# annegnx/PnP-Flow

Measured on AMD Instinct MI355X. Metric: restored images/sec, higher is better.
Workload: dtype f32-equivalent (f16 hi+lo split operands, 3 x f16 MFMA per product, f32 accumulate); 1 GPU; CelebA-shaped 256x256 box-inpainting (half-size 40, sigma 0.05) pnp_flow B=32/GPU 100x5 (the configuration BASELINE.json's metric is quoted on; main.py:132-136 at 256^2); image=256x256x3, batch_per_gpu=32, global_batch=32, steps_pnp=100, num_samples=5, weights=synthetic seed 0 (no checkpoint offline), hipgraph=True, unet_batch=160, parallelism=dp1 (contiguous shards of the global batch, no data-path collective)

## Files before the change

### pnpflow_amd/csrc/conv_sp.hip

```cpp
#include <cstdlib>
#include "pp_common.h"

namespace pf {

constexpr int SP_PITCH = 20, SP_PW = 18;
constexpr int sp_rows(int MT) { return 8 * MT; }
constexpr int sp_npix(int MT) { return (sp_rows(MT) + 2) * SP_PW; }
constexpr int sp_patch(int MT) { return (sp_rows(MT) + 2) * SP_PITCH * 64; }
constexpr int sp_a9(int MT) { return (sp_npix(MT) * 4 + 255) / 256; }
constexpr int sp_tap(int NT, int TERMS = 3) { return (TERMS == 3 ? 2 : 1) * NT * 1024; }
constexpr int sp_x(int NT, int TERMS = 3) { return (5 * sp_tap(NT, TERMS) + 4095) / 4096 * 4096; }
constexpr int sp_y(int NT, int TERMS = 3) { return 4 * sp_tap(NT, TERMS); }
constexpr int SP_TAB = PP_MAXCH * 32;
constexpr int sp_lds(int MT, int NT, int TERMS = 3) { return sp_x(NT, TERMS) + sp_y(NT, TERMS) + 2 * sp_patch(MT) + SP_TAB; }
constexpr int sp_stage_n(int A9, int tap) {
    const int slot = tap < 4 ? tap : tap < 8 ? tap - 1 : 7;
    if (tap == 4 || tap == 8) return 0;
    return A9 / 7 + (slot < A9 % 7 ? 1 : 0);
}
constexpr int sp_stage_0(int A9, int tap) { int n = 0; for (int t = 0; t < tap; ++t) n += sp_stage_n(A9, t); return n; }

__device__ __forceinline__ void glds16_sp(unsigned voff, const char* sbase, unsigned lds_dst) {
    unsigned keep;
    asm volatile("s_mov_b32 %0, m0\n\ts_mov_b32 m0, %3\n\ts_nop 0\n\tglobal_load_lds_dwordx4 %1, %2\n\ts_mov_b32 m0, %0"
                 : "=&s"(keep) : "v"(voff), "s"(sbase), "s"(lds_dst) : "memory");
}

#ifdef PP_PROBE_BUILD
__device__ unsigned long long* g_sp_dbg = nullptr;
#define SP_STAMP(k) do { if (stamp_buf != nullptr && blockIdx.x == 0 && tid == 0 && stamp_n < 64) stamp_buf[stamp_n * 16 + (k)] = __builtin_readcyclecounter(); } while (0)
#else
#define SP_STAMP(k) do { } while (0)
#endif

template <int MT, int NT, bool RES, int TERMS = 3>
__global__ __launch_bounds__(256, 1) void conv_sp_kernel(const PPParams p) {
    constexpr int TH = sp_rows(MT), NPIX = sp_npix(MT), A9 = sp_a9(MT), PATCH = sp_patch(MT);
    constexpr int TAPB = sp_tap(NT, TERMS), XB = sp_x(NT, TERMS), COUT = 32 * NT, OB = COUT * 4;
    constexpr int NFRAG = (TERMS == 3 ? 2 : 1) * (MT + NT), NMMA = TERMS * MT * NT;
    static_assert(TERMS == 3 || TERMS == 1, "split terms");
    static_assert(sp_y(NT, TERMS) % 4096 == 0 && 9 * TAPB >= XB, "refill rounds of 4 KiB; slot X's over-fetch stays inside the chunk image");
    constexpr int REQ1 = sp_stage_0(A9, 4), REQ2 = A9 - REQ1 + 3;
    static_assert(sp_stage_0(A9, 9) == A9 && REQ1 + NT + 4 * MT * NT < 64, "staging distribution / vmcnt range");
    extern __shared__ __attribute__((aligned(16))) char smem[];
    const int tid = threadIdx.x;
    const int lane = tid & 63, wq = __builtin_amdgcn_readfirstlane(tid >> 6);
    const int l31 = lane & 31, hi = lane >> 5;
    constexpr unsigned PATCH0 = (unsigned)(XB + sp_y(NT, TERMS)), TAB = PATCH0 + 2u * (unsigned)PATCH;
    const pp_float_cptr scale_c = (pp_float_cptr)(uintptr_t)p.scale;
    const int nch = p.n9;

    const int qi = tid & 3, p0 = tid >> 2;
    unsigned pk[A9], ldsw[A9];
#pragma unroll
    for (int i = 0; i < A9; ++i) {
        const int pp = min(p0 + 64 * i, NPIX - 1);
        const int py = pp / SP_PW, px = pp - py * SP_PW;
        pk[i] = (unsigned)(py * p.W + px) | ((py == 0 ? 1u : 0u) << 20) | ((py == TH + 1 ? 1u : 0u) << 21) | ((px == 0 ? 1u : 0u) << 22) |
                ((px == SP_PW - 1 ? 1u : 0u) << 23);
        ldsw[i] = PATCH0 + (unsigned)((py * SP_PITCH + px) * 64) + (unsigned)((((qi >> 1) ^ ((px >> 2) & 3)) << 4) + (qi & 1) * 8);
    }
    const int pix_safe = p.W + 1;

    const int prow = l31 >> 4, pcol = l31 & 15;
    unsigned a_addr[3][2];
// ... 20 lines not shown
    const int rot = ntl > 0 ? (int)(((long)rg * p.rot) % ntl) : 0;
    auto tile_of = [&](int it) __attribute__((always_inline)) -> PPTile {
        const int idx = min(it, ntl - 1);
        const int wrapped = idx + rot >= ntl ? idx + rot - ntl : idx + rot;
        const int tl = t_begin + wrapped;
        PPTile r;
        const int tx = tl & ((1 << p.lx) - 1), ty = (tl >> p.lx) & ((1 << p.ly) - 1);
        r.b = tl >> (p.lx + p.ly); r.oy0 = ty * TH; r.ox0 = tx * 16;
        r.edge = (ty == 0 ? 1 : 0) | (ty == (1 << p.ly) - 1 ? 2 : 0) | (tx == 0 ? 4 : 0) | (tx == (1 << p.lx) - 1 ? 8 : 0);
        return r;
    };

    float4 ra[A9];
    unsigned zero_v;
    asm volatile("v_mov_b32 %0, 0" : "=v"(zero_v));
    struct Coef { float4 csc, csh; float ascale; unsigned inval; };
    Coef cf0, cf1;
    typedef const __attribute__((address_space(1))) char* gptr;
    struct Src { gptr base; unsigned cs4; };
    const unsigned q16 = (unsigned)qi * 16u;
    struct Desc { gptr base; const char* cb; unsigned cs4; int edge; unsigned sofs; };
    struct Ent { uint4 a, b; };
    auto fetch = [&](int c) __attribute__((always_inline)) -> Ent {
        Ent e;
        e.a = *reinterpret_cast<const uint4*>(smem + TAB + (unsigned)c * 32u); e.b = *reinterpret_cast<const uint4*>(smem + TAB + (unsigned)c * 32u + 16u);
        return e;
    };
    auto sptr = [&](unsigned lo, unsigned hi) __attribute__((always_inline)) -> gptr {
        return (gptr)(((unsigned long long)(unsigned)__builtin_amdgcn_readfirstlane((int)hi) << 32) | (unsigned)__builtin_amdgcn_readfirstlane((int)lo));
    };
    auto describe = [&](const PPTile& tl, const Ent& e) __attribute__((always_inline)) -> Desc {
        const int pix = (tl.b * p.H + tl.oy0) * p.W + tl.ox0 - p.W - 1;
        const int cstride = __builtin_amdgcn_readfirstlane((int)e.b.x), coff = __builtin_amdgcn_readfirstlane((int)e.b.y);
        const int gn_c0 = __builtin_amdgcn_readfirstlane((int)e.b.z), seg = __builtin_amdgcn_readfirstlane((int)e.b.w);
        Desc d;
        d.sofs = (unsigned)(8 * tl.b + seg) * 4u;
        d.edge = tl.edge;
        d.cb = reinterpret_cast<const char*>(p.coef + (tl.b * 2 * p.coef_stride + gn_c0));
        d.base = sptr(e.a.x, e.a.y) + (long)(pix * cstride + coff) * 4;
        d.cs4 = (unsigned)cstride * 4u;
        return d;
    };
    auto prep = [&](Coef& N, const Desc& d) __attribute__((always_inline)) -> Src {
        N.ascale = *reinterpret_cast<const float*>(reinterpret_cast<const char*>(p.scale) + d.sofs + zero_v);
        unsigned inval = 0;
#pragma unroll
        for (int i = 0; i < A9; ++i) inval |= (((pk[i] >> 20) & (unsigned)d.edge) != 0u ? 1u : 0u) << i;
        N.inval = inval;
        N.csc = *reinterpret_cast<const float4*>(d.cb + q16); N.csh = *reinterpret_cast<const float4*>(d.cb + (unsigned)(p.coef_stride * 4) + q16);
        Src r; r.base = d.base; r.cs4 = d.cs4;
        return r;
    };
    auto issue_one = [&](const Coef& N, const Src& sr, int i) __attribute__((always_inline)) {
        const unsigned px = ((N.inval >> i) & 1u) ? (unsigned)pix_safe : (pk[i] & 0xffffu);
        const pp_f4v t_ = *reinterpret_cast<const __attribute__((address_space(1))) pp_f4v*>(sr.base + (__umul24(px, sr.cs4) + q16));
        ra[i] = make_float4(t_.x, t_.y, t_.z, t_.w);
    };
    auto transform_one = [&](const Coef& S, int i, unsigned pofs) __attribute__((always_inline)) {
        float4 v = ra[i];
        v.x = silu_pp(v.x * S.csc.x + S.csh.x); v.y = silu_pp(v.y * S.csc.y + S.csh.y);
        v.z = silu_pp(v.z * S.csc.z + S.csh.z); v.w = silu_pp(v.w * S.csc.w + S.csh.w);
        const float f = ((S.inval >> i) & 1u) ? 0.0f : S.ascale;
        v.x *= f; v.y *= f; v.z *= f; v.w *= f;
        f16x4 h = {(_Float16)v.x, (_Float16)v.y, (_Float16)v.z, (_Float16)v.w};
        if constexpr (TERMS == 3) {
            f16x4 l = {(_Float16)(v.x - (float)h[0]), (_Float16)(v.y - (float)h[1]), (_Float16)(v.z - (float)h[2]), (_Float16)(v.w - (float)h[3])};
            const unsigned addr = ldsw[i] + pofs;
            *reinterpret_cast<f16x4*>(smem + addr) = h;
            *reinterpret_cast<f16x4*>(smem + (addr ^ 32u)) = l;
        } else {
            *reinterpret_cast<f16x4*>(smem + ldsw[i] + pofs) = h;
        }
    };

    f32x16 acc[MT][NT];
#pragma unroll
    for (int mt = 0; mt < MT; ++mt)
#pragma unroll
        for (int nt = 0; nt < NT; ++nt)
#pragma unroll
            for (int r = 0; r < 16; ++r) acc[mt][nt][r] = 0.f;
    float run1[4 * NT], run2[4 * NT];
#pragma unroll
    for (int j = 0; j < 4 * NT; ++j) { run1[j] = 0.f; run2[j] = 0.f; }
    int run_b = -1, run_n = 0;

    auto flush_stats = [&]() __attribute__((always_inline)) {
// ... 82 lines not shown
    auto load_tap = [&](int set, int tap, unsigned pofs) __attribute__((always_inline)) {
        const int ky = tap / 3, kx = tap % 3;
        const unsigned wb = (unsigned)(tap < 5 ? tap * TAPB : XB + (tap - 5) * TAPB) + b_lane;
        if constexpr (TERMS == 3) {
#pragma unroll
            for (int mt = 0; mt < MT; ++mt) fa[set][mt][1] = *reinterpret_cast<const f16x8*>(smem + a_addr[kx][1] + (unsigned)((mt * 2 + ky) * SP_PITCH * 64) + pofs);
        }
#pragma unroll
        for (int nt = 0; nt < NT; ++nt) fb[set][nt][0] = *reinterpret_cast<const f16x8*>(smem + wb + (unsigned)(nt * 1024));
#pragma unroll
        for (int mt = 0; mt < MT; ++mt) fa[set][mt][0] = *reinterpret_cast<const f16x8*>(smem + a_addr[kx][0] + (unsigned)((mt * 2 + ky) * SP_PITCH * 64) + pofs);
        if constexpr (TERMS == 3) {
#pragma unroll
            for (int nt = 0; nt < NT; ++nt) fb[set][nt][1] = *reinterpret_cast<const f16x8*>(smem + wb + (unsigned)(NT * 1024 + nt * 1024));
        }
    };
    auto load_frag = [&](int set, int tap, unsigned pofs, int idx) __attribute__((always_inline)) {
        const int ky = tap / 3, kx = tap % 3;
        const unsigned wb = (unsigned)(tap < 5 ? tap * TAPB : XB + (tap - 5) * TAPB) + b_lane;
        if constexpr (TERMS == 3) {
            if (idx < MT) fa[set][idx][1] = *reinterpret_cast<const f16x8*>(smem + a_addr[kx][1] + (unsigned)((idx * 2 + ky) * SP_PITCH * 64) + pofs);
            else if (idx < MT + NT) fb[set][idx - MT][0] = *reinterpret_cast<const f16x8*>(smem + wb + (unsigned)((idx - MT) * 1024));
            else if (idx < 2 * MT + NT) fa[set][idx - MT - NT][0] = *reinterpret_cast<const f16x8*>(smem + a_addr[kx][0] + (unsigned)(((idx - MT - NT) * 2 + ky) * SP_PITCH * 64) + pofs);
            else fb[set][idx - 2 * MT - NT][1] = *reinterpret_cast<const f16x8*>(smem + wb + (unsigned)(NT * 1024 + (idx - 2 * MT - NT) * 1024));
        } else {
            if (idx < NT) fb[set][idx][0] = *reinterpret_cast<const f16x8*>(smem + wb + (unsigned)(idx * 1024));
            else fa[set][idx - NT][0] = *reinterpret_cast<const f16x8*>(smem + a_addr[kx][0] + (unsigned)(((idx - NT) * 2 + ky) * SP_PITCH * 64) + pofs);
        }
    };
    auto mma_group = [&](int set, int g) __attribute__((always_inline)) {
// ... 45 lines not shown
                acc[mt][nt] = __builtin_amdgcn_mfma_f32_32x32x16_f16(fa[set][mt][term == 0 ? 1 : 0], fb[set][nt][term == 1 ? 1 : 0], acc[mt][nt], 0, 0, 0);
                __builtin_amdgcn_sched_barrier(0);
                const int j = g * NT + nt;
                if (j < nrounds) {
                    if ((j & 3) == 0) asm volatile("s_mov_b32 m0, %0\n\ts_nop 0" :: "s"(dst0 + (unsigned)(j * 1024)) : "memory");
                    if ((j & 3) == 0) asm volatile("global_load_lds_dwordx4 %0, %1" :: "v"(b_lane), "s"(sb + j * 1024) : "memory");
                    if ((j & 3) == 1) asm volatile("global_load_lds_dwordx4 %0, %1 offset:1024" :: "v"(b_lane), "s"(sb + (j - 1) * 1024) : "memory");
                    if ((j & 3) == 2) asm volatile("global_load_lds_dwordx4 %0, %1 offset:2048" :: "v"(b_lane), "s"(sb + (j - 2) * 1024) : "memory");
                    if ((j & 3) == 3) asm volatile("global_load_lds_dwordx4 %0, %1 offset:3072" :: "v"(b_lane), "s"(sb + (j - 3) * 1024) : "memory");
                }
                if (j < NFRAG) load_frag(nset, ntap, npofs, j);
                __builtin_amdgcn_sched_barrier(0);
            }
        }
        asm volatile("s_mov_b32 m0, %0" :: "s"(keep));
    };

    int stamp_n = 0; (void)stamp_n;
#ifdef PP_PROBE_BUILD
    unsigned long long* const stamp_buf = g_sp_dbg;
#endif
    gptr wimg_next = (gptr)(uintptr_t)p.ch[1].wimg;
    Desc dn;
    Src sr;
    auto chunk = [&](int it, int c, auto SI_, bool last_chunk) __attribute__((always_inline)) {
        constexpr int SI = decltype(SI_)::value;
        constexpr unsigned PCUR = SI ? PATCH : 0, PNXT = SI ? 0 : PATCH;
        Coef& C = SI == 0 ? cf1 : cf0;
        Coef& N = SI == 0 ? cf0 : cf1;
        const gptr wnext = wimg_next;
// ... 15 lines not shown
        else asm volatile("s_waitcnt vmcnt(%0) lgkmcnt(0)" :: "n"(REQ1) : "memory");
#pragma unroll
        for (int i = REQ1; i < A9; ++i) asm volatile("" :: "v"(ra[i].x));
        SP_STAMP(13);
        __builtin_amdgcn_s_barrier();
        __builtin_amdgcn_sched_barrier(0);
        SP_STAMP(5);
        mma_tap_refill((4 + SI) & 1, wnext, 0, XB / 4096, (5 + SI) & 1, 5, PCUR);
        SP_STAMP(6);
#pragma unroll
        for (int tap = 5; tap < 8; ++tap) {
            __builtin_amdgcn_sched_barrier(0);
            int q = c + 3, wrap = 0;
            if (q >= nch) { q -= nch; wrap = 1; }
            if (q >= nch) { q -= nch; wrap = 2; }
            const int c2 = c + 2 >= nch ? c + 2 - nch : c + 2;
            Ent eq, e2;
            if (tap == 6) { eq = fetch(q); e2 = fetch(c2); }
            load_tap((tap + 1 + SI) & 1, tap + 1, PCUR);
#pragma unroll
            for (int i = sp_stage_0(A9, tap); i < sp_stage_0(A9, tap) + sp_stage_n(A9, tap); ++i) { transform_one(C, i, PNXT); issue_one(N, sr, i); }
            if (tap == 6) {
                dn = describe(tile_of(it + wrap), eq);
                wimg_next = sptr(e2.a.z, e2.a.w);
            }
            if (tap == 7) sr = prep(C, dn);
            mma_tap((tap + SI) & 1);
            tap_pattern();
            __builtin_amdgcn_sched_barrier(0);
            SP_STAMP(2 + tap);
        }
        __builtin_amdgcn_sched_barrier(0);
        asm volatile("s_waitcnt vmcnt(%0) lgkmcnt(0)" :: "n"(REQ2) : "memory");
#pragma unroll
        for (int i = 0; i < REQ1; ++i) asm volatile("" :: "v"(ra[i].x));
        SP_STAMP(14);
        __builtin_amdgcn_s_barrier();
        __builtin_amdgcn_sched_barrier(0);
        SP_STAMP(10);
        mma_tap_refill((8 + SI) & 1, wnext, 5, 4 * TAPB / 4096, (9 + SI) & 1, 0, PNXT);
        SP_STAMP(11);
        SP_STAMP(12);
        ++stamp_n;
    };

    if (ntl <= 0) return;
    for (int c = 0; c < nch; ++c) {
        if (tid == 0) {
            const unsigned long long sp_ = (unsigned long long)(uintptr_t)p.ch[c].src, wp_ = (unsigned long long)(uintptr_t)p.ch[c].wimg;
            *reinterpret_cast<uint4*>(smem + TAB + (unsigned)c * 32u) = make_uint4((unsigned)sp_, (unsigned)(sp_ >> 32), (unsigned)wp_, (unsigned)(wp_ >> 32));
            *reinterpret_cast<uint4*>(smem + TAB + (unsigned)c * 32u + 16u) = make_uint4((unsigned)p.ch[c].cstride, (unsigned)p.ch[c].coff, (unsigned)p.ch[c].gn_c0, (unsigned)p.ch[c].seg);
        }
    }
    __syncthreads();
    {
        const Src s0 = prep(cf0, describe(tile_of(0), fetch(0)));
#pragma unroll
        for (int i = 0; i < A9; ++i) issue_one(cf0, s0, i);
        {
            const char* w0 = reinterpret_cast<const char*>(p.ch[0].wimg);
#pragma unroll
            for (int j = 0; j < (TERMS == 3 ? 9 * TAPB : XB) / 4096; ++j) glds16_sp(dma_lane, w0 + j * 4096, (unsigned)(j * 4096) + (unsigned)(wq * 1024));
            if constexpr (TERMS != 3) {
#pragma unroll
                for (int j = 0; j < 4 * TAPB / 4096; ++j) glds16_sp(dma_lane, w0 + 5 * TAPB + j * 4096, (unsigned)(XB + j * 4096) + (unsigned)(wq * 1024));
            }
        }
#pragma unroll
        for (int i = 0; i < A9; ++i) transform_one(cf0, i, 0);
        const Src s1 = prep(cf1, describe(tile_of(0), fetch(1)));
#pragma unroll
        for (int i = 0; i < A9; ++i) issue_one(cf1, s1, i);
        sr = prep(cf0, describe(tile_of(2 >= nch ? 1 : 0), fetch(2 >= nch ? 2 - nch : 2)));
        asm volatile("s_waitcnt vmcnt(0) lgkmcnt(0)" ::: "memory");
        __builtin_amdgcn_s_barrier();
        __builtin_amdgcn_sched_barrier(0);
        load_tap(0, 0, 0);
    }
    const int seg_lo[4] = {0, seg_c1 > 0 ? seg_c1 : nch, seg_c2 > 0 ? seg_c2 : nch, nch};
#pragma unroll 1
    for (int it = 0; it < ntl; ++it) {
        tile_inputs(tile_of(it));
#pragma unroll 1
        for (int sg = 0; sg < 3; ++sg) {
            const int lo = seg_lo[sg], hi = seg_lo[sg + 1];
            if (lo >= hi) continue;
            if (sg > 0) {
                const PPTile tl = tile_of(it);
                const float ratio = scale_c[8 * tl.b + seg_id[sg]] * scale_c[8 * tl.b + 4 + seg_id[sg - 1]];
                if (ratio != 1.0f) {
#pragma unroll
                    for (int mt = 0; mt < MT; ++mt)
#pragma unroll
                        for (int nt = 0; nt < NT; ++nt)
#pragma unroll
                            for (int r = 0; r < 16; ++r) acc[mt][nt][r] *= ratio;
                }
// ... 4 lines not shown
                chunk(it, c + 1, ic<1>{}, false);
            }
        }
        epilogue(tile_of(it));
    }
    flush_stats();
    asm volatile("s_waitcnt vmcnt(0)" ::: "memory");
}


static int ilog2_exact_sp(int v) { int l = 0; while ((1 << l) < v) ++l; return (1 << l) == v ? l : -1; }

bool conv_sp_supported(const ConvParams& p, int stride, int up, int terms) {
    static const int mode = getenv("PNPFLOW_HIP_SP") ? atoi(getenv("PNPFLOW_HIP_SP")) : 1;
    if (mode == 0 || (terms != 3 && !(terms == 1 && mode != 3)) || stride != 1 || up != 0 || p.gnb_x != nullptr) return false;
    if (p.Cout != 128 && !(p.Cout == 64 && mode == 1)) return false;
    if (p.out_cstride != p.Cout || (p.residual != nullptr && p.res_cstride != p.Cout)) return false;
    if (p.addvec == nullptr) return false;
    const int TH = p.Cout == 128 ? sp_rows(2) : sp_rows(4);
    if (p.H % TH || p.W % 16 || p.Hs != p.H || p.Ws != p.W) return false;
    if ((TH + 1) * p.W + SP_PW - 1 > 65535) return false;
    if (ilog2_exact_sp(p.H / TH) < 0 || ilog2_exact_sp(p.W / 16) < 0) return false;
    const int grid = persistent_grid();
    if (grid < 8 || (long)p.B * (p.H / TH) * (p.W / 16) < 4L * grid) return false;
    int nch = 0;
    for (int i = 0; i < p.nseg; ++i) {
        const ConvSeg& s = p.seg[i];
        if ((double)p.B * p.H * p.W * s.cstride >= 2147483648.0) return false;
        if (s.w_mode != 0 || s.w16 == nullptr || s.C % 32 || s.taps != 9 || s.xform != 2) return false;
        nch += s.C / 16;
    }
    if (nch < 2 || nch > PP_MAXCH || (nch & 1)) return false;
    return p.gn_C > 0 && p.coef != nullptr && p.scale != nullptr;
}

template <int MT, int NT, int TERMS>
static hipError_t launch_sp_t(const PPParams& p0, hipStream_t s) {
    static unsigned long long attr_set[2] = {0ull, 0ull};
    const bool res = p0.residual != nullptr;
    const void* kern = res ? reinterpret_cast<const void*>(conv_sp_kernel<MT, NT, true, TERMS>) : reinterpret_cast<const void*>(conv_sp_kernel<MT, NT, false, TERMS>);
    { hipError_t e = set_max_dynamic_lds_once(kern, attr_set[res ? 1 : 0], 160 * 1024); if (e != hipSuccess) return e; }
    const int grid = persistent_grid();
    if (grid <= 0) return hipErrorInvalidConfiguration;
    PPParams p = p0;
    p.lx = ilog2_exact_sp(p.W / 16); p.ly = ilog2_exact_sp(p.H / sp_rows(MT));
    p.rot = 5;
    if (res) hipLaunchKernelGGL((conv_sp_kernel<MT, NT, true, TERMS>), dim3(grid), dim3(256), sp_lds(MT, NT, TERMS), s, p);
    else hipLaunchKernelGGL((conv_sp_kernel<MT, NT, false, TERMS>), dim3(grid), dim3(256), sp_lds(MT, NT, TERMS), s, p);
    return hipGetLastError();
}

hipError_t launch_conv_sp(const PPParams& p0, hipStream_t s, int terms) {
    if (p0.n9 < 2 || (p0.n9 & 1) || p0.n1 != 0 || (terms != 3 && terms != 1)) return hipErrorInvalidValue;
    if (p0.cout == 128) return terms == 3 ? launch_sp_t<2, 4, 3>(p0, s) : launch_sp_t<2, 4, 1>(p0, s);
    if (p0.cout == 64) return terms == 3 ? launch_sp_t<4, 2, 3>(p0, s) : launch_sp_t<4, 2, 1>(p0, s);
    return hipErrorInvalidValue;
}

}
```

### pnpflow_amd/csrc/engine.hip

```cpp
#include <algorithm>
#include <cmath>
#include <cstdio>
#include <cstring>
#include <cstdlib>
#include <functional>
#include <map>
#include <memory>
#include <string>
#include <vector>

#include "../../include/pnpflow_hip.h"
#include "pf_common.h"
#include "weight_pack.h"

using namespace pf;

namespace {

struct HostTensor { std::vector<int64_t> shape; std::vector<float> data; bool loaded = false; };

struct ResDesc {
    std::string prefix;
    int cin0 = 0, cin1 = 0;
    int cout = 0;
// ... 408 lines not shown
    if (!sp && !(p.Cout == 32 && conv_pp_supported(p, stride, up, terms))) return 0;
    q = PPParams{};
    q.cout = p.Cout;
    const int kc = sp ? 16 : 32;
    int n = 0;
    for (int i = 0; i < p.nseg; ++i) {
        const ConvSeg& sg = p.seg[i];
        auto it = e->w16_src.find(sg.w16);
        if (it == e->w16_src.end()) return 0;
        for (int cc = 0; cc < sg.C / kc; ++cc) {
            PPChunk& k = q.ch[n++];
            k.src = sg.src; k.cstride = sg.cstride; k.coff = sg.coff + cc * kc; k.xform = sg.xform;
            k.gn_c0 = sg.gn_off + cc * kc; k.seg = i;
            const std::string& wn = it->second.name; const int lo = it->second.lo + cc * kc;
            const wpack::Oihw w = oihw(e, wn);
            if (w.O != p.Cout || (sp && w.kk != 9)) return 0;
            k.wimg = !sp ? weight_image(e, wn + "#pp" + std::to_string(lo), [&] { return wpack::chunk_pp(w, lo); })
                         : weight_image(e, wn + (terms == 1 ? "#sph" : "#sp") + std::to_string(p.Cout) + "_" + std::to_string(lo), [&] { return wpack::chunk_sp(w, lo, p.Cout / 32, terms); });
            if (!k.wimg) return 0;
            (sg.taps == 9 ? q.n9 : q.n1) += 1;
        }
    }
    q.B = p.B; q.H = p.H; q.W = p.W;
    q.out = p.out; q.addvec = p.addvec; q.addvec_bs = p.addvec_bs; q.residual = p.residual; q.res_scale = p.res_scale;
    q.stats_out = p.stats_out; q.out_scale = p.out_scale; q.coef = p.coef; q.coef_stride = p.coef_stride; q.scale = p.scale;
    return sp ? 2 : 1;
}

static void push_conv(Builder& bd, const ConvParams& p0, int stride = 1, int up = 0) {
    ConvParams p = with_coef(bd, p0, bd.plan->ops);
    Op op{}; op.kind = OP_CONV; op.terms = conv_terms(bd.e);
    op.use_pp = attach_pp(bd, p, stride, up, op.ppp);
// ... 1435 lines not shown

int pf_engine_profile_read(pf_engine* e, int64_t* launches, double* ms_conv_gemm, double* flops_conv_gemm) {
    if (!e) return PF_ERR_INVALID;
    HIPCHK(e, hipDeviceSynchronize());
    FILE* dump = getenv("PNPFLOW_HIP_PROFILE_CSV") ? fopen(getenv("PNPFLOW_HIP_PROFILE_CSV"), "w") : nullptr;
    if (dump) fprintf(dump, "idx,H,W,Cout,K,nseg,taps0,stride,up,gflop,us,tflops,dma,alg_mb\n");
    for (size_t i = 0; i < e->ev_used; ++i) {
        float ms = 0.f;
        if (hipEventElapsedTime(&ms, e->ev_pool[i].first, e->ev_pool[i].second) == hipSuccess) { e->prof_ms += ms; e->prof_launches += 1; }
        if (dump && i < e->ev_ops.size() && e->ev_ops[i]) {
            const Op& op = *e->ev_ops[i]; size_t K = 0;
            for (int j = 0; j < op.cp.nseg; ++j) K += (size_t)op.cp.seg[j].taps * op.cp.seg[j].C;
            double bytes = (double)op.cp.B * op.cp.H * op.cp.W * op.cp.Cout * 4.0 * (op.cp.residual ? 2.0 : 1.0);
            for (int j = 0; j < op.cp.nseg; ++j) bytes += (double)op.cp.B * op.cp.Hs * op.cp.Ws * op.cp.seg[j].C * 4.0;
            fprintf(dump, "%zu,%d,%d,%d,%zu,%d,%d,%d,%d,%.4f,%.2f,%.2f,%d,%.3f", i, op.cp.H, op.cp.W, op.cp.Cout, K, op.cp.nseg, op.cp.seg[0].taps,
                    op.stride, op.up, op.flops / 1e9, ms * 1e3, op.flops / (ms * 1e-3) / 1e12, op.use_pp == 2 ? 5 : op.use_pp ? 2 : op.dma, bytes / 1e6);
            fprintf(dump, "\n");
        }
    }
    if (dump) fclose(dump);
    e->ev_used = 0;
    if (launches) *launches = e->prof_launches;
    if (ms_conv_gemm) *ms_conv_gemm = e->prof_ms;
    if (flops_conv_gemm) *flops_conv_gemm = e->prof_flops;
    return PF_OK;
}

}

#include "engine_dflow.inc"
```

### pnpflow_amd/csrc/pf_common.h

```cpp
#pragma once
#include <hip/hip_runtime.h>
#include <stdint.h>
#include <atomic>

namespace pf {

inline hipError_t set_max_dynamic_lds_once(const void* kernel, unsigned long long& done, int bytes = 160 * 1024) {
    int dev = 0;
    hipError_t e = hipGetDevice(&dev);
    if (e != hipSuccess) return e;
    if (dev >= 0 && dev < 64 && ((done >> dev) & 1ull)) return hipSuccess;
    e = hipFuncSetAttribute(kernel, hipFuncAttributeMaxDynamicSharedMemorySize, bytes);
    if (e == hipSuccess && dev >= 0 && dev < 64) done |= 1ull << dev;
    return e;
}

inline int device_cu_count() {
    static std::atomic<int> cache[64] = {};
    int dev = 0;
    if (hipGetDevice(&dev) != hipSuccess) return 0;
    if (dev >= 0 && dev < 64) { const int c = cache[dev].load(std::memory_order_relaxed); if (c > 0) return c; }
    int v = 0;
    if (hipDeviceGetAttribute(&v, hipDeviceAttributeMultiprocessorCount, dev) != hipSuccess || v < 0) v = 0;
    if (dev >= 0 && dev < 64) cache[dev].store(v, std::memory_order_relaxed);
// ... 109 lines not shown
hipError_t launch_gn_coef(const GnCoefParams& p, int B, hipStream_t s);

struct PrepParams {
    const float* src[3]; void* dst[3];
    int C[3], cstride[3], coff[3], xform[3], gn_off[3];
    int nseg, B, Hs, Ws, terms;
    const float* coef; int coef_stride;
    const float* scale;
};
hipError_t launch_prep_split(const PrepParams& p, hipStream_t s);
bool conv_dma_supported(const ConvParams& p, int stride, int up, int terms);
bool conv_dma_phase_shape_ok(const ConvParams& p, int terms);
hipError_t launch_conv_dma(const ConvParams& p, int up, hipStream_t s, int terms);
size_t conv_dma_a16_bytes(int B, int C, int Hs, int Ws, int terms);

constexpr int PP_MAXCH = 24;
struct PPChunk {
    const float* src;
    const void* wimg;
    int cstride, coff;
    int xform;
    int gn_c0;
    int seg;
    int pad_;
};
struct PPParams {
    PPChunk ch[PP_MAXCH];
    int n9, n1;
    int cout;
    int B, H, W, lx, ly;
    int rot;
// ... 102 lines not shown
```

### pnpflow_amd/csrc/weight_pack.h

```cpp
#pragma once
#include <cstddef>
#include <vector>

namespace wpack {

using half_t = _Float16;
constexpr int KC = 16;

struct Oihw {
    const float* w; int O, I, kk;
    float operator()(int o, int i, int tap) const { return w[((size_t)o * I + i) * kk + tap]; }
};

struct Split { half_t hi, lo; half_t part(int p) const { return p ? lo : hi; } };
inline Split split16(float w) { w *= 256.0f; const half_t hi = (half_t)w; return {hi, (half_t)(w - (float)hi)}; }

inline int col_channel(int n) { return 4 * (n & 7) + (n >> 3); }

inline std::vector<float> frag32(const Oihw& w, int lo, int hi) {
    const int C = hi - lo, nchunk = (C + KC - 1) / KC;
    std::vector<float> img((size_t)nchunk * w.kk * w.O * KC, 0.f);
    for (int c = 0; c < C; ++c)
        for (int tap = 0; tap < w.kk; ++tap)
            for (int n = 0; n < w.O; ++n)
// ... 27 lines not shown
}

inline std::vector<half_t> chunk_sp(const Oihw& w, int lo, int NT, int terms) {
    const int P = terms == 1 ? 1 : 2;
    std::vector<half_t> img((size_t)w.kk * P * NT * 512, (half_t)0.f);
    size_t at = 0;
    for (int tap = 0; tap < w.kk; ++tap)
        for (int part = 0; part < P; ++part)
            for (int nt = 0; nt < NT; ++nt)
                for (int kh = 0; kh < 2; ++kh)
                    for (int n = 0; n < 32; ++n)
                        for (int i = 0; i < 8; ++i) img[at++] = split16(w(32 * nt + col_channel(n), lo + 8 * kh + i, tap)).part(part);
    return img;
}

inline std::vector<half_t> edge_frag(const Oihw& w, bool begin) {
    const int cimg = begin ? w.I : w.O;
    std::vector<half_t> img((size_t)2 * 2 * 64 * 8, (half_t)0.f);
    for (int ks = 0; ks < 2; ++ks) for (int hh = 0; hh < 2; ++hh) for (int n = 0; n < 32; ++n) for (int j = 0; j < 8; ++j) {
        const int k = begin ? 16 * ks + 8 * hh + j : n;
        if (k >= 9 * cimg) continue;
        const Split s = begin ? split16(w(n, k / 9, k % 9)) : split16(w(n % cimg, 16 * hh + 8 * ks + j, n / cimg));
        for (int part = 0; part < 2; ++part) img[((((size_t)ks * 2 + part) * 2 + hh) * 32 + n) * 8 + j] = s.part(part);
    }
    return img;
}

inline std::vector<float> adjoint(const Oihw& w, int lo, int hi) {
    const int C = hi - lo;
    std::vector<float> t((size_t)C * w.O * w.kk);
// ... 21 lines not shown
```

Baseline: 3.300 images/s.

## Fuse 1x1 shortcut conv into the streaming 3x3 conv kernel

Adds a shortcut-carrying variant of the persistent 3x3 conv kernel. It appends the 1x1 shortcut segment's raw-input chunks after the 3x3 chunks, which extends the ResNet block fusion so the shortcut conv no longer needs a separate pass or launch. The 1x1 weights stream through an LDS ring. Raw inputs skip the GN/SiLU transform through a per-chunk flag, and the accumulator is rescaled between segments. Small global-to-LDS touch loads are issued during the 3x3 taps, apparently to prefetch shortcut inputs into cache. This adds LDS use, kernel complexity and a rescaling step that can affect precision.

Measured after the change: 3.307 images/s (median of 6 runs). About the same (+0.2%).

```diff
diff --git a/pnpflow_amd/csrc/conv_sp.hip b/pnpflow_amd/csrc/conv_sp.hip
--- a/pnpflow_amd/csrc/conv_sp.hip
+++ b/pnpflow_amd/csrc/conv_sp.hip
@@ -13,6 +13,12 @@
 constexpr int sp_y(int NT, int TERMS = 3) { return 4 * sp_tap(NT, TERMS); }
 constexpr int SP_TAB = PP_MAXCH * 32;
 constexpr int sp_lds(int MT, int NT, int TERMS = 3) { return sp_x(NT, TERMS) + sp_y(NT, TERMS) + 2 * sp_patch(MT) + SP_TAB; }
+constexpr int SP_RING = 4, SP_TOUCH = 1024;
+constexpr int sp_lds_sc(int MT, int NT) { return sp_lds(MT, NT, 3) + SP_RING * sp_tap(NT, 3) + SP_TOUCH; }
+#ifndef SP_TOUCH_PAIRS_N
+#define SP_TOUCH_PAIRS_N 2
+#endif
+constexpr int SP_TOUCH_PAIRS = SP_TOUCH_PAIRS_N;
 constexpr int sp_stage_n(int A9, int tap) {
     const int slot = tap < 4 ? tap : tap < 8 ? tap - 1 : 7;
     if (tap == 4 || tap == 8) return 0;
@@ -25,30 +31,40 @@
     asm volatile("s_mov_b32 %0, m0\n\ts_mov_b32 m0, %3\n\ts_nop 0\n\tglobal_load_lds_dwordx4 %1, %2\n\ts_mov_b32 m0, %0"
                  : "=&s"(keep) : "v"(voff), "s"(sbase), "s"(lds_dst) : "memory");
 }
+__device__ __forceinline__ void glds4_sp(unsigned voff, const __attribute__((address_space(1))) char* sbase, unsigned lds_dst) {
+    unsigned keep;
+    asm volatile("s_mov_b32 %0, m0\n\ts_mov_b32 m0, %3\n\ts_nop 0\n\tglobal_load_lds_dword %1, %2\n\ts_mov_b32 m0, %0"
+                 : "=&s"(keep) : "v"(voff), "s"(sbase), "s"(lds_dst) : "memory");
+}
 
 #ifdef PP_PROBE_BUILD
 __device__ unsigned long long* g_sp_dbg = nullptr;
+__device__ int g_sp_touch_off = 0;
 #define SP_STAMP(k) do { if (stamp_buf != nullptr && blockIdx.x == 0 && tid == 0 && stamp_n < 64) stamp_buf[stamp_n * 16 + (k)] = __builtin_readcyclecounter(); } while (0)
 #else
 #define SP_STAMP(k) do { } while (0)
 #endif
 
-template <int MT, int NT, bool RES, int TERMS = 3>
+template <int MT, int NT, bool RES, int TERMS = 3, bool SC = false>
 __global__ __launch_bounds__(256, 1) void conv_sp_kernel(const PPParams p) {
+    static_assert(!SC || (TERMS == 3 && !RES), "the shortcut-carrying form: default precision, no identity residual");
     constexpr int TH = sp_rows(MT), NPIX = sp_npix(MT), A9 = sp_a9(MT), PATCH = sp_patch(MT);
     constexpr int TAPB = sp_tap(NT, TERMS), XB = sp_x(NT, TERMS), COUT = 32 * NT, OB = COUT * 4;
     constexpr int NFRAG = (TERMS == 3 ? 2 : 1) * (MT + NT), NMMA = TERMS * MT * NT;
     static_assert(TERMS == 3 || TERMS == 1, "split terms");
     static_assert(sp_y(NT, TERMS) % 4096 == 0 && 9 * TAPB >= XB, "refill rounds of 4 KiB; slot X's over-fetch stays inside the chunk image");
-    constexpr int REQ1 = sp_stage_0(A9, 4), REQ2 = A9 - REQ1 + 3;
+    constexpr int NTOUCH = SC ? SP_TOUCH_PAIRS * (TH * 16 / 256) : 0;
+    constexpr int REQ1 = sp_stage_0(A9, 4), REQ2 = A9 - REQ1 + 3 + NTOUCH;
     static_assert(sp_stage_0(A9, 9) == A9 && REQ1 + NT + 4 * MT * NT < 64, "staging distribution / vmcnt range");
     extern __shared__ __attribute__((aligned(16))) char smem[];
     const int tid = threadIdx.x;
     const int lane = tid & 63, wq = __builtin_amdgcn_readfirstlane(tid >> 6);
     const int l31 = lane & 31, hi = lane >> 5;
     constexpr unsigned PATCH0 = (unsigned)(XB + sp_y(NT, TERMS)), TAB = PATCH0 + 2u * (unsigned)PATCH;
+    constexpr unsigned W1 = TAB + (unsigned)SP_TAB, TOUCH = W1 + (unsigned)(SP_RING * TAPB);
     const pp_float_cptr scale_c = (pp_float_cptr)(uintptr_t)p.scale;
-    const int nch = p.n9;
+    const int n9 = p.n9;
+    const int nch = SC ? p.n9 + p.n1 : p.n9;
 
     const int qi = tid & 3, p0 = tid >> 2;
     unsigned pk[A9], ldsw[A9];
@@ -99,12 +115,12 @@
     float4 ra[A9];
     unsigned zero_v;
     asm volatile("v_mov_b32 %0, 0" : "=v"(zero_v));
-    struct Coef { float4 csc, csh; float ascale; unsigned inval; };
+    struct Coef { float4 csc, csh; float ascale; unsigned inval; float lk; };
     Coef cf0, cf1;
     typedef const __attribute__((address_space(1))) char* gptr;
     struct Src { gptr base; unsigned cs4; };
     const unsigned q16 = (unsigned)qi * 16u;
-    struct Desc { gptr base; const char* cb; unsigned cs4; int edge; unsigned sofs; };
+    struct Desc { gptr base; const char* cb; unsigned cs4; int edge; unsigned sofs; int raw; };
     struct Ent { uint4 a, b; };
     auto fetch = [&](int c) __attribute__((always_inline)) -> Ent {
         Ent e;
@@ -117,8 +133,10 @@
     auto describe = [&](const PPTile& tl, const Ent& e) __attribute__((always_inline)) -> Desc {
         const int pix = (tl.b * p.H + tl.oy0) * p.W + tl.ox0 - p.W - 1;
         const int cstride = __builtin_amdgcn_readfirstlane((int)e.b.x), coff = __builtin_amdgcn_readfirstlane((int)e.b.y);
-        const int gn_c0 = __builtin_amdgcn_readfirstlane((int)e.b.z), seg = __builtin_amdgcn_readfirstlane((int)e.b.w);
+        const int gn_c0 = __builtin_amdgcn_readfirstlane((int)e.b.z), segw = __builtin_amdgcn_readfirstlane((int)e.b.w);
+        const int seg = SC ? (segw & 0xff) : segw;
         Desc d;
+        d.raw = SC ? (segw >> 8) & 1 : 0;
         d.sofs = (unsigned)(8 * tl.b + seg) * 4u;
         d.edge = tl.edge;
         d.cb = reinterpret_cast<const char*>(p.coef + (tl.b * 2 * p.coef_stride + gn_c0));
@@ -126,13 +144,20 @@
         d.cs4 = (unsigned)cstride * 4u;
         return d;
     };
-    auto prep = [&](Coef& N, const Desc& d) __attribute__((always_inline)) -> Src {
+    auto prep = [&](Coef& N, const Desc& d, auto SEL_) __attribute__((always_inline)) -> Src {
         N.ascale = *reinterpret_cast<const float*>(reinterpret_cast<const char*>(p.scale) + d.sofs + zero_v);
         unsigned inval = 0;
 #pragma unroll
         for (int i = 0; i < A9; ++i) inval |= (((pk[i] >> 20) & (unsigned)d.edge) != 0u ? 1u : 0u) << i;
         N.inval = inval;
         N.csc = *reinterpret_cast<const float4*>(d.cb + q16); N.csh = *reinterpret_cast<const float4*>(d.cb + (unsigned)(p.coef_stride * 4) + q16);
+        if constexpr (SC && decltype(SEL_)::value == 0) N.lk = 0.0f;
+        if constexpr (SC && decltype(SEL_)::value != 0) {
+            const bool rw = d.raw != 0;
+            N.csc.x = rw ? 1.0f : N.csc.x; N.csc.y = rw ? 1.0f : N.csc.y; N.csc.z = rw ? 1.0f : N.csc.z; N.csc.w = rw ? 1.0f : N.csc.w;
+            N.csh.x = rw ? 0.0f : N.csh.x; N.csh.y = rw ? 0.0f : N.csh.y; N.csh.z = rw ? 0.0f : N.csh.z; N.csh.w = rw ? 0.0f : N.csh.w;
+            N.lk = rw ? -__builtin_inff() : 0.0f;
+        }
         Src r; r.base = d.base; r.cs4 = d.cs4;
         return r;
     };
@@ -143,8 +168,14 @@
     };
     auto transform_one = [&](const Coef& S, int i, unsigned pofs) __attribute__((always_inline)) {
         float4 v = ra[i];
-        v.x = silu_pp(v.x * S.csc.x + S.csh.x); v.y = silu_pp(v.y * S.csc.y + S.csh.y);
-        v.z = silu_pp(v.z * S.csc.z + S.csh.z); v.w = silu_pp(v.w * S.csc.w + S.csh.w);
+        if constexpr (SC) {
+            auto silu_lk = [&](float u) __attribute__((always_inline)) -> float { return u * __builtin_amdgcn_rcpf(1.0f + __builtin_amdgcn_exp2f(__builtin_fmaf(u, -1.44269504088896340736f, S.lk))); };
+            v.x = silu_lk(v.x * S.csc.x + S.csh.x); v.y = silu_lk(v.y * S.csc.y + S.csh.y);
+            v.z = silu_lk(v.z * S.csc.z + S.csh.z); v.w = silu_lk(v.w * S.csc.w + S.csh.w);
+        } else {
+            v.x = silu_pp(v.x * S.csc.x + S.csh.x); v.y = silu_pp(v.y * S.csc.y + S.csh.y);
+            v.z = silu_pp(v.z * S.csc.z + S.csh.z); v.w = silu_pp(v.w * S.csc.w + S.csh.w);
+        }
         const float f = ((S.inval >> i) & 1u) ? 0.0f : S.ascale;
         v.x *= f; v.y *= f; v.z *= f; v.w *= f;
         f16x4 h = {(_Float16)v.x, (_Float16)v.y, (_Float16)v.z, (_Float16)v.w};
@@ -156,6 +187,17 @@
         } else {
             *reinterpret_cast<f16x4*>(smem + ldsw[i] + pofs) = h;
         }
+    };
+
+    auto transform_raw = [&](const Coef& S, int i, unsigned pofs) __attribute__((always_inline)) {
+        float4 v = ra[i];
+        const float f = ((S.inval >> i) & 1u) ? 0.0f : S.ascale;
+        v.x *= f; v.y *= f; v.z *= f; v.w *= f;
+        f16x4 h = {(_Float16)v.x, (_Float16)v.y, (_Float16)v.z, (_Float16)v.w};
+        f16x4 l = {(_Float16)(v.x - (float)h[0]), (_Float16)(v.y - (float)h[1]), (_Float16)(v.z - (float)h[2]), (_Float16)(v.w - (float)h[3])};
+        const unsigned addr = ldsw[i] + pofs;
+        *reinterpret_cast<f16x4*>(smem + addr) = h;
+        *reinterpret_cast<f16x4*>(smem + (addr ^ 32u)) = l;
     };
 
     f32x16 acc[MT][NT];
@@ -268,6 +310,17 @@
 #pragma unroll
             for (int nt = 0; nt < NT; ++nt) fb[set][nt][1] = *reinterpret_cast<const f16x8*>(smem + wb + (unsigned)(NT * 1024 + nt * 1024));
         }
+    };
+    auto load_tap1 = [&](int set, unsigned wslot, unsigned pofs) __attribute__((always_inline)) {
+        const unsigned wb = wslot + b_lane;
+#pragma unroll
+        for (int mt = 0; mt < MT; ++mt) fa[set][mt][1] = *reinterpret_cast<const f16x8*>(smem + a_addr[1][1] + (unsigned)((mt * 2 + 1) * SP_PITCH * 64) + pofs);
+#pragma unroll
+        for (int nt = 0; nt < NT; ++nt) fb[set][nt][0] = *reinterpret_cast<const f16x8*>(smem + wb + (unsigned)(nt * 1024));
+#pragma unroll
+        for (int mt = 0; mt < MT; ++mt) fa[set][mt][0] = *reinterpret_cast<const f16x8*>(smem + a_addr[1][0] + (unsigned)((mt * 2 + 1) * SP_PITCH * 64) + pofs);
+#pragma unroll
+        for (int nt = 0; nt < NT; ++nt) fb[set][nt][1] = *reinterpret_cast<const f16x8*>(smem + wb + (unsigned)(NT * 1024 + nt * 1024));
     };
     auto load_frag = [&](int set, int tap, unsigned pofs, int idx) __attribute__((always_inline)) {
         const int ky = tap / 3, kx = tap % 3;
@@ -343,6 +396,26 @@
             }
         }
         asm volatile("s_mov_b32 m0, %0" :: "s"(keep));
+    };
+
+    auto touch = [&](int it, int c) __attribute__((always_inline)) {
+        const PPTile tl = tile_of(it);
+        const int pix = (tl.b * p.H + tl.oy0) * p.W + tl.ox0;
+        const int last = (p.n1 >> 1) - 1;
+#pragma unroll
+        for (int k = 0; k < SP_TOUCH_PAIRS; ++k) {
+            const Ent e = fetch(n9 + 2 * min(1 + SP_TOUCH_PAIRS * c + k, last));
+            const int cstride = __builtin_amdgcn_readfirstlane((int)e.b.x), coff = __builtin_amdgcn_readfirstlane((int)e.b.y);
+            const gptr base = sptr(e.a.x, e.a.y) + (long)(pix * cstride + coff) * 4;
+#pragma unroll
+            for (int i = 0; i < TH * 16 / 256; ++i) {
+                unsigned voff = __umul24((unsigned)(((tid >> 4) + 16 * i) * p.W + (tid & 15)), (unsigned)cstride * 4u);
+#ifdef PP_PROBE_BUILD
+                if (g_sp_touch_off) voff = 0u;
+#endif
+                glds4_sp(voff, base, TOUCH + (unsigned)(wq * 256));
+            }
+        }
     };
 
     int stamp_n = 0; (void)stamp_n;
@@ -388,9 +461,10 @@
             int q = c + 3, wrap = 0;
             if (q >= nch) { q -= nch; wrap = 1; }
             if (q >= nch) { q -= nch; wrap = 2; }
-            const int c2 = c + 2 >= nch ? c + 2 - nch : c + 2;
+            const int c2 = c + 2 >= n9 ? c + 2 - n9 : c + 2;
             Ent eq, e2;
             if (tap == 6) { eq = fetch(q); e2 = fetch(c2); }
+            if constexpr (SC) { if (tap == 5) touch(it, c); }
             load_tap((tap + 1 + SI) & 1, tap + 1, PCUR);
 #pragma unroll
             for (int i = sp_stage_0(A9, tap); i < sp_stage_0(A9, tap) + sp_stage_n(A9, tap); ++i) { transform_one(C, i, PNXT); issue_one(N, sr, i); }
@@ -398,7 +472,7 @@
                 dn = describe(tile_of(it + wrap), eq);
                 wimg_next = sptr(e2.a.z, e2.a.w);
             }
-            if (tap == 7) sr = prep(C, dn);
+            if (tap == 7) sr = prep(C, dn, ic<1>{});
             mma_tap((tap + SI) & 1);
             tap_pattern();
             __builtin_amdgcn_sched_barrier(0);
@@ -418,17 +492,68 @@
         ++stamp_n;
     };
 
+    int ring_n = 0;
+    auto chunk1 = [&](int it, int g, auto SI_) __attribute__((always_inline)) {
+        constexpr int SI = decltype(SI_)::value;
+        constexpr unsigned PNXT = SI ? 0 : PATCH;
+        constexpr int NREG = 3 * MT * NT / 2;
+        Coef& C = SI == 0 ? cf1 : cf0;
+        Coef& N = SI == 0 ? cf0 : cf1;
+        static_assert(!SC || A9 + 2 <= NREG, "one float4 of the next chunk is staged per two MFMAs of the tap");
+        const bool next_raw = g + 1 < nch;
+        int q = g + 3, wrap = 0;
+        if (q >= nch) { q -= nch; wrap = 1; }
+        if (q >= nch) { q -= nch; wrap = 2; }
+        int jn = g - n9 + SP_RING;
+        if (jn >= p.n1) jn -= p.n1;
+        if (jn >= p.n1) jn -= p.n1;
+        Ent eq, ew;
+        SP_STAMP(0);
+#pragma unroll
+        for (int gi = 0; gi < NREG; ++gi) {
+            __builtin_amdgcn_sched_barrier(0);
+            if (gi == 0) { eq = fetch(q); ew = fetch(n9 + jn); }
+#pragma unroll
+            for (int k = 2 * gi; k < 2 * gi + 2; ++k) {
+                const int grp = k / NT, nt = k % NT, term = grp / MT, mt = grp % MT;
+                acc[mt][nt] = __builtin_amdgcn_mfma_f32_32x32x16_f16(fa[SI][mt][term == 0 ? 1 : 0], fb[SI][nt][term == 1 ? 1 : 0], acc[mt][nt], 0, 0, 0);
+            }
+            if (gi < A9) {
+                if (next_raw) transform_raw(C, gi, PNXT); else transform_one(C, gi, PNXT);
+                issue_one(N, sr, gi);
+            }
+            if (gi == A9) dn = describe(tile_of(it + wrap), eq);
+            if (gi == A9 + 1) sr = prep(C, dn, ic<0>{});
+            __builtin_amdgcn_sched_barrier(0);
+            SP_STAMP(1 + gi);
+        }
+        const gptr wsrc = sptr(ew.a.z, ew.a.w);
+        const unsigned slot = W1 + (unsigned)((ring_n & (SP_RING - 1)) * TAPB), slot_next = W1 + (unsigned)(((ring_n + 1) & (SP_RING - 1)) * TAPB);
+        ++ring_n;
+        asm volatile("s_waitcnt vmcnt(%0) lgkmcnt(0)" :: "n"(A9 + 3) : "memory");
+        SP_STAMP(13);
+        __builtin_amdgcn_s_barrier();
+        __builtin_amdgcn_sched_barrier(0);
+        SP_STAMP(14);
+#pragma unroll
+        for (int j = 0; j < TAPB / 4096; ++j) glds16_sp(dma_lane, (const char*)wsrc + j * 4096, slot + (unsigned)(j * 4096 + wq * 1024));
+        if (next_raw) load_tap1(SI ^ 1, slot_next, PNXT); else load_tap(SI ^ 1, 0, PNXT);
+        __builtin_amdgcn_sched_barrier(0);
+        ++stamp_n;
+    };
+
     if (ntl <= 0) return;
     for (int c = 0; c < nch; ++c) {
         if (tid == 0) {
             const unsigned long long sp_ = (unsigned long long)(uintptr_t)p.ch[c].src, wp_ = (unsigned long long)(uintptr_t)p.ch[c].wimg;
             *reinterpret_cast<uint4*>(smem + TAB + (unsigned)c * 32u) = make_uint4((unsigned)sp_, (unsigned)(sp_ >> 32), (unsigned)wp_, (unsigned)(wp_ >> 32));
-            *reinterpret_cast<uint4*>(smem + TAB + (unsigned)c * 32u + 16u) = make_uint4((unsigned)p.ch[c].cstride, (unsigned)p.ch[c].coff, (unsigned)p.ch[c].gn_c0, (unsigned)p.ch[c].seg);
+            *reinterpret_cast<uint4*>(smem + TAB + (unsigned)c * 32u + 16u) = make_uint4((unsigned)p.ch[c].cstride, (unsigned)p.ch[c].coff, (unsigned)p.ch[c].gn_c0,
+                                                                                         (unsigned)p.ch[c].seg | ((SC && p.ch[c].xform == 0) ? 0x100u : 0u));
         }
     }
     __syncthreads();
     {
-        const Src s0 = prep(cf0, describe(tile_of(0), fetch(0)));
+        const Src s0 = prep(cf0, describe(tile_of(0), fetch(0)), ic<1>{});
 #pragma unroll
         for (int i = 0; i < A9; ++i) issue_one(cf0, s0, i);
         {
@@ -439,13 +564,20 @@
 #pragma unroll
                 for (int j = 0; j < 4 * TAPB / 4096; ++j) glds16_sp(dma_lane, w0 + 5 * TAPB + j * 4096, (unsigned)(XB + j * 4096) + (unsigned)(wq * 1024));
             }
+            if constexpr (SC) {
+                for (int r = 0; r < SP_RING; ++r) {
+                    const char* w1 = reinterpret_cast<const char*>(p.ch[n9 + r % p.n1].wimg);
+#pragma unroll
+                    for (int j = 0; j < TAPB / 4096; ++j) glds16_sp(dma_lane, w1 + j * 4096, W1 + (unsigned)(r * TAPB + j * 4096) + (unsigned)(wq * 1024));
+                }
+            }
         }
 #pragma unroll
         for (int i = 0; i < A9; ++i) transform_one(cf0, i, 0);
-        const Src s1 = prep(cf1, describe(tile_of(0), fetch(1)));
+        const Src s1 = prep(cf1, describe(tile_of(0), fetch(1)), ic<1>{});
 #pragma unroll
         for (int i = 0; i < A9; ++i) issue_one(cf1, s1, i);
-        sr = prep(cf0, describe(tile_of(2 >= nch ? 1 : 0), fetch(2 >= nch ? 2 - nch : 2)));
+        sr = prep(cf0, describe(tile_of(2 >= nch ? 1 : 0), fetch(2 >= nch ? 2 - nch : 2)), ic<1>{});
         asm volatile("s_waitcnt vmcnt(0) lgkmcnt(0)" ::: "memory");
         __builtin_amdgcn_s_barrier();
         __builtin_amdgcn_sched_barrier(0);
@@ -455,6 +587,34 @@
 #pragma unroll 1
     for (int it = 0; it < ntl; ++it) {
         tile_inputs(tile_of(it));
+        if constexpr (SC) {
+#pragma unroll 1
+            for (int c = 0; c < n9; c += 2) {
+                chunk(it, c, ic<0>{}, false);
+                chunk(it, c + 1, ic<1>{}, false);
+            }
+            load_tap1(0, W1 + (unsigned)((ring_n & (SP_RING - 1)) * TAPB), 0);
+#pragma unroll 1
+            for (int sg = 1; sg < 3; ++sg) {
+                const int lo = sg == 1 ? seg_lo[1] : seg_lo[2], hi = sg == 1 ? seg_lo[2] : nch;
+                if (lo >= hi) continue;
+                const PPTile tl = tile_of(it);
+                const float ratio = scale_c[8 * tl.b + (sg == 1 ? seg_id[1] : seg_id[2])] * scale_c[8 * tl.b + 4 + (sg == 1 ? seg_id[0] : seg_id[1])];
+                if (ratio != 1.0f) {
+#pragma unroll
+                    for (int mt = 0; mt < MT; ++mt)
+#pragma unroll
+                        for (int nt = 0; nt < NT; ++nt)
+#pragma unroll
+                            for (int r = 0; r < 16; ++r) acc[mt][nt][r] *= ratio;
+                }
+#pragma unroll 1
+                for (int c = lo; c < hi; c += 2) {
+                    chunk1(it, c, ic<0>{});
+                    chunk1(it, c + 1, ic<1>{});
+                }
+            }
+        } else
 #pragma unroll 1
         for (int sg = 0; sg < 3; ++sg) {
             const int lo = seg_lo[sg], hi = seg_lo[sg + 1];
@@ -489,7 +649,7 @@
 bool conv_sp_supported(const ConvParams& p, int stride, int up, int terms) {
     static const int mode = getenv("PNPFLOW_HIP_SP") ? atoi(getenv("PNPFLOW_HIP_SP")) : 1;
     if (mode == 0 || (terms != 3 && !(terms == 1 && mode != 3)) || stride != 1 || up != 0 || p.gnb_x != nullptr) return false;
-    if (p.Cout != 128 && !(p.Cout == 64 && mode == 1)) return false;
+    if (p.Cout != 128 && !(p.Cout == 64 && (mode == 1 || mode == 3))) return false;
     if (p.out_cstride != p.Cout || (p.residual != nullptr && p.res_cstride != p.Cout)) return false;
     if (p.addvec == nullptr) return false;
     const int TH = p.Cout == 128 ? sp_rows(2) : sp_rows(4);
@@ -498,14 +658,20 @@
     if (ilog2_exact_sp(p.H / TH) < 0 || ilog2_exact_sp(p.W / 16) < 0) return false;
     const int grid = persistent_grid();
     if (grid < 8 || (long)p.B * (p.H / TH) * (p.W / 16) < 4L * grid) return false;
-    int nch = 0;
+    static const bool sc_on = !(getenv("PNPFLOW_HIP_SP_SC") && atoi(getenv("PNPFLOW_HIP_SP_SC")) == 0);
+    int nch = 0, n1 = 0;
     for (int i = 0; i < p.nseg; ++i) {
         const ConvSeg& s = p.seg[i];
         if ((double)p.B * p.H * p.W * s.cstride >= 2147483648.0) return false;
-        if (s.w_mode != 0 || s.w16 == nullptr || s.C % 32 || s.taps != 9 || s.xform != 2) return false;
-        nch += s.C / 16;
+        if (s.w_mode != 0 || s.w16 == nullptr || s.C % 32) return false;
+        if (s.taps == 9 && s.xform == 2 && n1 == 0) nch += s.C / 16;
+        else if (s.taps == 1 && s.xform == 0 && sc_on && terms == 3 && p.residual == nullptr && i > 0) {
+            if (s.cstride % 32 || s.coff % 32) return false;
+            n1 += s.C / 16;
+        } else return false;
     }
-    if (nch < 2 || nch > PP_MAXCH || (nch & 1)) return false;
+    if (nch < 2 || nch + n1 > PP_MAXCH || (nch & 1)) return false;
+    if (n1 > 0 && (p.seg[0].taps != 9 || p.seg[1].taps != 1 || nch < 4 || (SP_TOUCH_PAIRS > 0 && n1 / 2 - 1 > SP_TOUCH_PAIRS * nch))) return false;
     return p.gn_C > 0 && p.coef != nullptr && p.scale != nullptr;
 }
 
@@ -525,8 +691,26 @@
     return hipGetLastError();
 }
 
+template <int MT, int NT>
+static hipError_t launch_sp_sc(const PPParams& p0, hipStream_t s) {
+    static unsigned long long attr_set = 0ull;
+    const void* kern = reinterpret_cast<const void*>(conv_sp_kernel<MT, NT, false, 3, true>);
+    { hipError_t e = set_max_dynamic_lds_once(kern, attr_set, 160 * 1024); if (e != hipSuccess) return e; }
+    const int grid = persistent_grid();
+    if (grid <= 0) return hipErrorInvalidConfiguration;
+    PPParams p = p0;
+    p.lx = ilog2_exact_sp(p.W / 16); p.ly = ilog2_exact_sp(p.H / sp_rows(MT));
+    p.rot = 5;
+    hipLaunchKernelGGL((conv_sp_kernel<MT, NT, false, 3, true>), dim3(grid), dim3(256), sp_lds_sc(MT, NT), s, p);
+    return hipGetLastError();
+}
+
 hipError_t launch_conv_sp(const PPParams& p0, hipStream_t s, int terms) {
-    if (p0.n9 < 2 || (p0.n9 & 1) || p0.n1 != 0 || (terms != 3 && terms != 1)) return hipErrorInvalidValue;
+    if (p0.n9 < 2 || (p0.n9 & 1) || (p0.n1 & 1) || p0.n9 + p0.n1 > PP_MAXCH || (terms != 3 && terms != 1)) return hipErrorInvalidValue;
+    if (p0.n1 != 0) {
+        if (terms != 3 || p0.residual != nullptr || p0.n9 < 4 || (SP_TOUCH_PAIRS > 0 && p0.n1 / 2 - 1 > SP_TOUCH_PAIRS * p0.n9)) return hipErrorInvalidValue;
+        return p0.cout == 128 ? launch_sp_sc<2, 4>(p0, s) : p0.cout == 64 ? launch_sp_sc<4, 2>(p0, s) : hipErrorInvalidValue;
+    }
     if (p0.cout == 128) return terms == 3 ? launch_sp_t<2, 4, 3>(p0, s) : launch_sp_t<2, 4, 1>(p0, s);
     if (p0.cout == 64) return terms == 3 ? launch_sp_t<4, 2, 3>(p0, s) : launch_sp_t<4, 2, 1>(p0, s);
     return hipErrorInvalidValue;
diff --git a/pnpflow_amd/csrc/engine.hip b/pnpflow_amd/csrc/engine.hip
--- a/pnpflow_amd/csrc/engine.hip
+++ b/pnpflow_amd/csrc/engine.hip
@@ -446,8 +446,9 @@
             k.gn_c0 = sg.gn_off + cc * kc; k.seg = i;
             const std::string& wn = it->second.name; const int lo = it->second.lo + cc * kc;
             const wpack::Oihw w = oihw(e, wn);
-            if (w.O != p.Cout || (sp && w.kk != 9)) return 0;
+            if (w.O != p.Cout || (sp && w.kk != sg.taps)) return 0;
             k.wimg = !sp ? weight_image(e, wn + "#pp" + std::to_string(lo), [&] { return wpack::chunk_pp(w, lo); })
+                   : sg.taps == 1 ? weight_image(e, wn + "#sp1_" + std::to_string(p.Cout) + "_" + std::to_string(lo), [&] { return wpack::chunk_sp_tap1(w, lo, p.Cout / 32); })
                          : weight_image(e, wn + (terms == 1 ? "#sph" : "#sp") + std::to_string(p.Cout) + "_" + std::to_string(lo), [&] { return wpack::chunk_sp(w, lo, p.Cout / 32, terms); });
             if (!k.wimg) return 0;
             (sg.taps == 9 ? q.n9 : q.n1) += 1;
@@ -1913,7 +1914,7 @@
             double bytes = (double)op.cp.B * op.cp.H * op.cp.W * op.cp.Cout * 4.0 * (op.cp.residual ? 2.0 : 1.0);
             for (int j = 0; j < op.cp.nseg; ++j) bytes += (double)op.cp.B * op.cp.Hs * op.cp.Ws * op.cp.seg[j].C * 4.0;
             fprintf(dump, "%zu,%d,%d,%d,%zu,%d,%d,%d,%d,%.4f,%.2f,%.2f,%d,%.3f", i, op.cp.H, op.cp.W, op.cp.Cout, K, op.cp.nseg, op.cp.seg[0].taps,
-                    op.stride, op.up, op.flops / 1e9, ms * 1e3, op.flops / (ms * 1e-3) / 1e12, op.use_pp == 2 ? 5 : op.use_pp ? 2 : op.dma, bytes / 1e6);
+                    op.stride, op.up, op.flops / 1e9, ms * 1e3, op.flops / (ms * 1e-3) / 1e12, op.use_pp == 2 ? (op.ppp.n1 > 0 ? 6 : 5) : op.use_pp ? 2 : op.dma, bytes / 1e6);
             fprintf(dump, "\n");
         }
     }
diff --git a/pnpflow_amd/csrc/pf_common.h b/pnpflow_amd/csrc/pf_common.h
--- a/pnpflow_amd/csrc/pf_common.h
+++ b/pnpflow_amd/csrc/pf_common.h
@@ -147,7 +147,7 @@
 hipError_t launch_conv_dma(const ConvParams& p, int up, hipStream_t s, int terms);
 size_t conv_dma_a16_bytes(int B, int C, int Hs, int Ws, int terms);
 
-constexpr int PP_MAXCH = 24;
+constexpr int PP_MAXCH = 32;
 struct PPChunk {
     const float* src;
     const void* wimg;
diff --git a/pnpflow_amd/csrc/weight_pack.h b/pnpflow_amd/csrc/weight_pack.h
--- a/pnpflow_amd/csrc/weight_pack.h
+++ b/pnpflow_amd/csrc/weight_pack.h
@@ -65,6 +65,11 @@
     return img;
 }
 
+inline std::vector<half_t> chunk_sp_tap1(const Oihw& w, int lo, int NT) {
+    if (w.kk != 1) return {};
+    return chunk_sp(w, lo, NT, 3);
+}
+
 inline std::vector<half_t> edge_frag(const Oihw& w, bool begin) {
     const int cimg = begin ? w.I : w.O;
     std::vector<half_t> img((size_t)2 * 2 * 64 * 8, (half_t)0.f);
```
